# barc4/barc4dip

Measured on AMD Instinct MI355X. Metric: frames/s (2048×2048 fp32) through FFT→PSD→autocorr; % HBM roofline, higher is better.
Workload: dtype f32

## Files before the change

### barc4dip_amd/csrc/b4d_colpass.hip

```cpp
#define B4D_UNIT_TAG 1
#define B4D_UNIT_PASSES 2
#include "b4d_passes.hpp"

namespace b4d {
int col_psd_ac_pass(const b4d_plan* pl, const ColArgs& a, int batch, hipStream_t st) {
    return dispatch_col<COL_PSD_AC>(pl, a, batch, st);
}
}
```

### barc4dip_amd/csrc/b4d_common.hpp

```cpp
#pragma once
#include <hip/hip_runtime.h>

#include <atomic>
#include <mutex>
#include <string>

#include "../../include/b4d.h"

namespace b4d {

std::string& last_error();
inline int fail(int code, const std::string& msg) {
    last_error() = msg;
    return code;
}
int get_scratch(size_t bytes, void** out, hipStream_t stream);
std::recursive_mutex& scratch_mutex();
#define B4D_SCRATCH_LOCK() std::lock_guard<std::recursive_mutex> b4d_scratch_lk__(::b4d::scratch_mutex())

extern std::atomic<int> g_opt_track_predict;
extern std::atomic<int> g_opt_lanes;
extern std::atomic<int> g_opt_exp;

int ensure_dynamic_lds(const void* kernel, size_t bytes);
int lane_stream(int idx, hipStream_t* out);

#define B4D_HIP(call)                                                                      \
    do {                                                                                   \
        hipError_t e__ = (call);                                                           \
        if (e__ != hipSuccess)                                                             \
            return ::b4d::fail(B4D_EHIP, std::string(#call) + ": " + hipGetErrorString(e__)); \
    } while (0)

}
```

### barc4dip_amd/csrc/b4d_fft2d.hpp

```cpp
#pragma once
#include <hip/hip_runtime.h>

#include <algorithm>
#include <cmath>
#include <cstdint>
#include <mutex>
#include <string>
#include <vector>

#include "../../include/b4d.h"
#include "b4d_common.hpp"
#include "b4d_fft.hpp"
#include "b4d_peak.hpp"

#ifndef B4D_UNIT_TAG
#define B4D_UNIT_TAG 0
#endif
#define B4D_PASS_R2C 1
#define B4D_PASS_COL 2
#define B4D_PASS_NYQ 4
#define B4D_PASS_C2R 8
#ifndef B4D_UNIT_PASSES
#define B4D_UNIT_PASSES (B4D_PASS_R2C | B4D_PASS_COL | B4D_PASS_NYQ | B4D_PASS_C2R)
#endif
// ... 28 lines not shown
        c.x *= inv;
        c.y *= inv;
    }
    return c;
}

struct RowSrc {
    int frame, y0, y1, x0, x1;
    float mean, denom;
    int pad;
};

#ifndef B4D_K1_ITER
#define B4D_K1_ITER 1
#endif
template <int NX, int SEQ, bool SRC, int ITER = 1>
__global__ void __launch_bounds__((NX / E16) * SEQ)
k_row_r2c(const float* __restrict__ in, float2* __restrict__ spec, float* __restrict__ nyq_rows,
          const float2* __restrict__ tw, int ny, int ct_w, const RowSrc* __restrict__ srcs) {
    using G = RowGeom<NX>;
    constexpr int T = G::T, E = E16;
    constexpr bool WV = T <= 64;
    static_assert(ITER == 1 || !SRC, "ROI sources run one group per workgroup");
    __shared__ float2 lds_all[SEQ * G::LDS_ELEMS];
    const int seq = threadIdx.x / T, u = threadIdx.x % T;
    const size_t frame = blockIdx.y;
    if (SRC) {
        const int wa = 2 * blockIdx.x * SEQ, wb = wa + 2 * SEQ;
        if (wb <= srcs[frame].y0 || wa >= srcs[frame].y1) return;
    }
    float2* lds = lds_all + seq * G::LDS_ELEMS;
    float2 va[ITER][E];
#pragma unroll
    for (int it = 0; it < ITER; ++it) {
        float2(&v)[E] = va[it];
        const int pair = (blockIdx.x * ITER + it) * SEQ + seq;
        const bool live = 2 * pair < ny;
        if (!live) {
// ... 2 lines not shown
        } else if (SRC) {
            const RowSrc sd = srcs[frame];
            const int ya = 2 * pair, yb = ya + 1;
            const bool ina = ya >= sd.y0 && ya < sd.y1, inb = yb >= sd.y0 && yb < sd.y1;
            const float* r0 = in + ((size_t)sd.frame * ny + ya) * NX;
            const float* r1 = r0 + NX;
            const float inv = 1.0f / sd.denom;
#pragma unroll
            for (int j = 0; j < E; ++j) {
                const int x = u + T * j;
                const bool inx = x >= sd.x0 && x < sd.x1;
                v[j].x = (ina && inx) ? (r0[x] - sd.mean) * inv : 0.f;
                v[j].y = (inb && inx) ? (r1[x] - sd.mean) * inv : 0.f;
            }
        } else {
            const float* r0 = in + (frame * ny + 2 * (size_t)pair) * NX;
            const float* r1 = r0 + NX;
#pragma unroll
            for (int j = 0; j < E; ++j) v[j] = make_float2(r0[u + T * j], r1[u + T * j]);
        }
    }
    const int nt = (NX / 2) / ct_w;
#pragma unroll
    for (int it = 0; it < ITER; ++it) {
        float2(&v)[E] = va[it];
        const int pair = (blockIdx.x * ITER + it) * SEQ + seq;
        const bool live = 2 * pair < ny;
        if (it > 0) fft_sync<WV>();
        Fft3<G, 1, WV>::run(v, v, u, 0, lds, tw);
        fft_sync<WV>();
#pragma unroll
        for (int j = 0; j < E; ++j) lds[u + T * j] = v[j];
        fft_sync<WV>();
        if (live) {
#pragma unroll
            for (int j = 0; j < E / 2; ++j) {
                const int k = u + T * j;
                const float2 z = v[j], zr = lds[(NX - k) & (NX - 1)];
                float2 a = make_float2(0.5f * (z.x + zr.x), 0.5f * (z.y - zr.y));
                float2 b = make_float2(0.5f * (z.y + zr.y), 0.5f * (zr.x - z.x));
                if (k == 0) {
                    const float2 zn = lds[NX / 2];
                    a = make_float2(z.x, 0.f);
                    b = make_float2(z.y, 0.f);
                    nyq_rows[frame * ny + 2 * pair] = zn.x;
                    nyq_rows[frame * ny + 2 * pair + 1] = zn.y;
                }
                const size_t o = spec_index(frame, nt, ny, ct_w, 2 * pair, k);
                spec[o] = a;
                spec[o + ct_w] = b;
            }
        }
    }
}

enum ColMode { COL_PSD_AC = 0, COL_FORWARD = 2 };

struct ColArgs {
    float2* spec;
    float* psd;
    const float2* tw;
    const float2* tw_inv;
    float psd_scale;
    int nx;
    unsigned flags;
// ... 11 lines not shown
        unsigned long long t__;                                                                   \
        asm volatile("s_memtime %0\n\ts_waitcnt lgkmcnt(0)" : "=s"(t__)::"memory");              \
        __builtin_amdgcn_sched_barrier(0);                                                        \
        if (p.diag && threadIdx.x == 0) p.diag[((size_t)blockIdx.y * gridDim.x + blockIdx.x) * 8 + (i)] = t__; \
    } while (0)
#ifdef B4D_DIAG_DRAIN
#define B4D_DRAIN() asm volatile("s_waitcnt vmcnt(0)" ::: "memory")
#else
#define B4D_DRAIN() do {} while (0)
#endif
#else
#define B4D_STAMP(i) do {} while (0)
#define B4D_DRAIN() do {} while (0)
#endif

template <int NY, int SPLIT = 1>
struct ColCfg {
    static constexpr int NC = 2;
    static constexpr int CPT = (NY == 4096 ? 4 : 8) / SPLIT;
    static constexpr int CT = NC * CPT * SPLIT;
    static constexpr int THREADS = CPT * (NY / E16);
    static constexpr int WAVES_PER_EU = THREADS >= 256 ? 4 : 1;
    using G = ColGeom<NY, CPT>;
    static constexpr int SB = 1;
    static constexpr size_t LDS_BYTES = sizeof(float2) * (size_t)G::LDS_ELEMS * CPT * SB;
    static constexpr bool SERIAL = true;
};

struct __attribute__((packed, aligned(4))) float4_u {
    float x, y, z, w;
};

typedef float f32x2 __attribute__((ext_vector_type(2)));
typedef float f32x4 __attribute__((ext_vector_type(4)));
// ... 13 lines not shown
}

template <int NC>
__device__ __forceinline__ void store_cols(f32x2 B4D_GLOBAL* rowp, const float2 (&c)[NC]) {
#pragma unroll
    for (int h = 0; h < NC / 2; ++h)
        *(f32x4 B4D_GLOBAL*)(rowp + 2 * h) = f32x4{c[2 * h].x, c[2 * h].y, c[2 * h + 1].x, c[2 * h + 1].y};
}
template <int NC>
__device__ __forceinline__ void store_cols(float2* __restrict__ rowp, const float2 (&c)[NC]) {
#pragma unroll
    for (int h = 0; h < NC / 2; ++h)
        *reinterpret_cast<float4*>(rowp + 2 * h) = make_float4(c[2 * h].x, c[2 * h].y, c[2 * h + 1].x, c[2 * h + 1].y);
}

template <int NY, int MODE, int SPLIT = 1, int UNIT = 0>
__global__ void __launch_bounds__((ColCfg<NY, SPLIT>::THREADS), (ColCfg<NY, SPLIT>::WAVES_PER_EU)) k_col(ColArgs p) {
    using Cfg = ColCfg<NY, SPLIT>;
    using G = typename Cfg::G;
    constexpr int T = G::T, E = E16, NC = Cfg::NC, CPT = Cfg::CPT, CT = Cfg::CT;
    extern __shared__ __attribute__((aligned(16))) float2 lds[];
    const int cp = threadIdx.x % CPT, u = threadIdx.x / CPT;
    const int nt = gridDim.x / SPLIT;
    int slot, fr;
    if (gridDim.y % 8 == 0) {
        const unsigned lin = blockIdx.x + gridDim.x * blockIdx.y, k = lin / 8;
        fr = 8 * (k / gridDim.x) + lin % 8;
        slot = k % gridDim.x;
    } else {
        slot = (nt % 8 == 0) ? (blockIdx.x % 8) * (nt * SPLIT / 8) + blockIdx.x / 8 : blockIdx.x;
        fr = blockIdx.y;
    }
    const int ct = slot / SPLIT;
    const int cpm = cp + CPT * (slot % SPLIT);
    const size_t frame = fr;
    const int nx = p.nx;
    float2* tile = p.spec + ((frame * nt + ct) * (size_t)NY) * CT;
    const unsigned toff = (unsigned)u * CT + NC * cpm;
    float2 v[NC][E];
    B4D_STAMP(0);
    int ry0 = 0, ry1 = NY;
    if (MODE == COL_FORWARD && p.srcs) {
        ry0 = p.srcs[fr].y0;
        ry1 = p.srcs[fr].y1;
    }
#pragma unroll
    for (int h = 0; h < NC / 2; ++h) {
#pragma unroll
// ... 3 lines not shown
                float4 q = *reinterpret_cast<const float4*>(tile + (size_t)kc * CT + NC * cpm + 2 * h);
                if (ky < ry0 || ky >= ry1) q = make_float4(0.f, 0.f, 0.f, 0.f);
                v[2 * h][j] = make_float2(q.x, q.y);
                v[2 * h + 1][j] = make_float2(q.z, q.w);
            } else {
                const f32x4 q = *at_bytes<f32x4>(sgpr_base(tile + (size_t)(T * j * CT) + 2 * h), toff * 8u);
                v[2 * h][j] = make_float2(q.x, q.y);
                v[2 * h + 1][j] = make_float2(q.z, q.w);
            }
        }
    }
    B4D_DRAIN();
    B4D_STAMP(1);
    Fft3<G, 1>::template run_sets<NC, Cfg::SERIAL, MODE != COL_PSD_AC, Cfg::SB>(v, u, cp, lds, p.tw);
    B4D_STAMP(2);
    const int kx0 = ct * CT + NC * cpm;

    if (MODE == COL_FORWARD) {
        unsigned toff3 = toff;
        asm volatile("" : "+v"(toff3));
#pragma unroll
        for (int j = 0; j < E; ++j) {
            float2 c[NC];
#pragma unroll
            for (int k = 0; k < NC; ++k) c[k] = v[k][j];
            store_cols<NC>(tile + (size_t)(T * j * CT) + toff3, c);
        }
        return;
    }

    const float s = p.psd_scale;
    float* psd = p.psd ? p.psd + frame * (size_t)NY * nx : nullptr;
    int uu = u;
    asm volatile("" : "+v"(uu));
    float2 w[NC / 2][E];
    constexpr int B3 = E / G::R3;
#pragma unroll
    for (int a = 0; a < B3; ++a) {
#pragma unroll
        for (int k = 0; k < NC; ++k) Fft3<G, 1>::stage3_one(v[k], a);
#pragma unroll
        for (int q = 0; q < G::R3; ++q) {
            const int j = a + B3 * q;
            const int ky = uu + T * j;
            float pw[NC];
#pragma unroll
            for (int k = 0; k < NC; ++k) pw[k] = v[k][j].x * v[k][j].x + v[k][j].y * v[k][j].y;
#ifdef B4D_EXP_PSD_TILED
            if (psd) {
                float* pt = psd + ((size_t)ct * NY + ky) * 32 + NC * cpm;
                *reinterpret_cast<float2*>(pt) = make_float2(pw[0] * s, pw[1] * s);
                *reinterpret_cast<float2*>(pt + 16) = make_float2(pw[1] * s, pw[0] * s);
            }
            if (false) {
#else
            if (psd) {
#endif
                const unsigned rd = (unsigned)((ky + NY / 2) & (NY - 1)) * nx, rm = (unsigned)((NY / 2 - ky) & (NY - 1)) * nx;
                if (NC == 4)
                    *reinterpret_cast<float4*>(&psd[rd + nx / 2 + kx0]) =
                        make_float4(pw[0] * s, pw[1] * s, pw[2 % NC] * s, pw[3 % NC] * s);
                else
                    *at_bytes<f32x2>(psd, (rd + nx / 2 + kx0) * 4u) = f32x2{pw[0] * s, pw[1] * s};
                if (NC == 4 && kx0 >= 1) {
                    float4_u m;
                    m.x = pw[3 % NC] * s;
                    m.y = pw[2 % NC] * s;
                    m.z = pw[1] * s;
                    m.w = pw[0] * s;
                    *reinterpret_cast<float4_u*>(&psd[rm + nx / 2 - kx0 - 3]) = m;
                } else {
#if defined(B4D_EXP_NOMIRROR)
#elif defined(B4D_EXP_ALIGNED_MIRROR)
// ... 7 lines not shown
                    if (cpm == 0 && kx0 >= 1) psd[rm + nx / 2 - kx0] = pw[0] * s;
#else
                    const unsigned mo = (rm + nx / 2 - kx0 - 1) * 4u;
                    *at_bytes<float>(psd, mo) = pw[1] * s;
                    if (kx0 >= 1) *at_bytes<float>(psd, mo + 4u) = pw[0] * s;
#endif
                }
            }
#pragma unroll
            for (int h = 0; h < NC / 2; ++h) w[h][j] = make_float2(pw[2 * h + 1], pw[2 * h]);
        }
    }
    B4D_STAMP(3);
    B4D_DRAIN();
    B4D_STAMP(4);
    if (kx0 == 0 && uu == 0 && (p.flags & B4D_REMOVE_MEAN)) w[0][0].y = 0.f;
    const float2* tw2 = p.tw_inv;
    int tid2 = threadIdx.x;
    asm volatile("" : "+v"(tid2));
    const int cp2 = tid2 % CPT, u2 = tid2 / CPT;
    const unsigned toff2 = (unsigned)u2 * CT + NC * (cp2 + CPT * (slot % SPLIT));
    __syncthreads();
    Fft3<G, 1>::template run_sets<NC / 2, Cfg::SERIAL, true, Cfg::SB>(w, u2, cp2, lds, tw2);
    B4D_STAMP(5);
    float2 vr[NC / 2][E];
    constexpr int SETE = G::LDS_ELEMS * CPT;
#pragma unroll
    for (int b = 0; b < NC / 2; b += Cfg::SB) {
        __syncthreads();
#pragma unroll
        for (int h = b; h < b + Cfg::SB; ++h)
// ... 2 lines not shown
        __syncthreads();
#pragma unroll
        for (int h = b; h < b + Cfg::SB; ++h)
#pragma unroll
            for (int j = 0; j < E; ++j) vr[h][j] = lds[(h - b) * SETE + ((NY - (u2 + T * j)) & (NY - 1)) * CPT + cp2];
    }
#pragma unroll
    for (int j = 0; j < E; ++j) {
        float2 c[NC];
#pragma unroll
        for (int h = 0; h < NC / 2; ++h) {
            const float2 z = make_float2(w[h][j].y, w[h][j].x), zr = vr[h][j];
            c[2 * h] = make_float2(0.5f * (z.x + zr.x), 0.5f * (z.y - zr.y));
            c[2 * h + 1] = make_float2(0.5f * (z.y + zr.y), 0.5f * (zr.x - z.x));
        }
        if (!p.half_rows || u2 + T * j <= NY / 2 + 1) {
            static_assert(NC == 2, "one 16-byte store per row");
            __builtin_nontemporal_store(f32x4{c[0].x, c[0].y, c[1].x, c[1].y},
                                        (f32x4 B4D_GLOBAL*)at_bytes<f32x2>(sgpr_base(tile + (size_t)(T * j * CT)), toff2 * 8u));
        }
    }
    B4D_STAMP(6);
    B4D_DRAIN();
    B4D_STAMP(7);
}

enum NyqMode { NYQ_PSD_AC = 0, NYQ_FORWARD = 2, NYQ_PROD = 3, NYQ_PROD_WHITEN = 4 };

struct NyqArgs {
    const float* rows;
    float2* f_out;
// ... 76 lines not shown
    const float2* tw;
    float scale;
    int ny, ct_w;
    unsigned flags;
    float* part_val;
    int* part_idx;
    unsigned* selw;
    int sel_stride;
    unsigned pred_bin;
    float* compact;
    int half;
    int nomap;
    int nblk;
    const unsigned* gate;
    int gate_stride;
};

enum RowOutMode { C2R_OUT = 0, C2R_PEAK = 1, C2R_MAG = 2, C2R_ROWS = 3 };

template <int NX, int SEQ, int MODE, int UNIT = 0>
__global__ void __launch_bounds__((NX / E16) * SEQ) k_row_c2r(RowOutArgs p) {
    using G = RowGeom<NX>;
    constexpr int T = G::T, E = E16;
    constexpr bool WV = T <= 64;
    __shared__ float2 lds_all[SEQ * G::LDS_ELEMS];
    const int seq = threadIdx.x / T, u = threadIdx.x % T;
    const size_t frame = blockIdx.y;
    const int ny = p.ny, ct_w = p.ct_w, nt = (NX / 2) / ct_w;
    if (MODE == C2R_MAG && p.gate && p.gate[frame * p.gate_stride]) return;
    int peak_pair = 0;
    if (MODE == C2R_ROWS) {
        float bv = -1.0f;
        int bi = 0x7fffffff;
        for (int i = threadIdx.x; i < p.nblk; i += T * SEQ) argmax_merge(bv, bi, p.part_val[frame * p.nblk + i], p.part_idx[frame * p.nblk + i]);
#pragma unroll
        for (int o = 32; o > 0; o >>= 1) {
// ... 7 lines not shown
            sv[threadIdx.x >> 6] = bv;
            si[threadIdx.x >> 6] = bi;
        }
        __syncthreads();
        bv = sv[0];
        bi = si[0];
        for (int i = 1; i < (T * SEQ + 63) / 64; ++i) argmax_merge(bv, bi, sv[i], si[i]);
        __syncthreads();
        const int yr = bi == 0x7fffffff ? 0 : bi / NX;
        peak_pair = ((yr + ny / 2) & (ny - 1)) >> 1;
    }
    const int nblk = gridDim.x, bx = blockIdx.x;
    const int pair = MODE == C2R_PEAK   ? 0
                     : MODE == C2R_ROWS ? (peak_pair + ny / 2 - 1 + min(bx * SEQ + seq, 2)) % (ny / 2)
                                        : bx * SEQ + seq;
    const bool live = (MODE == C2R_OUT && p.half) ? 2 * pair <= ny / 2 : 2 * pair < ny;
    const int yl = live ? 2 * pair : 0;
    float2* lds = lds_all + seq * G::LDS_ELEMS;
    float2 v[E];
#pragma unroll
    for (int j = 0; j < E / 2; ++j) {
        const int k = u + T * j;
        const size_t o = MODE == C2R_MAG ? spec_index_pow2(frame, nt, ny, ct_w, yl, k) : spec_index(frame, nt, ny, ct_w, yl, k);
        const f32x2 a_ = __builtin_nontemporal_load(reinterpret_cast<const f32x2*>(p.g + o)),
                    b_ = __builtin_nontemporal_load(reinterpret_cast<const f32x2*>(p.g + o + ct_w));
        const float2 a = make_float2(a_.x, a_.y), b = make_float2(b_.x, b_.y);
        if (k == 0) {
            v[j] = make_float2(b.x, a.x);
            lds[NX / 2] = make_float2(p.gnyq[frame * ny + yl + 1], p.gnyq[frame * ny + yl]);
        } else {
            v[j] = make_float2(a.y + b.x, a.x - b.y);
            lds[NX - k] = make_float2(b.x - a.y, a.x + b.y);
        }
    }
    fft_sync<WV>();
#pragma unroll
    for (int j = E / 2; j < E; ++j) v[j] = lds[u + T * j];
    fft_sync<WV>();
    Fft3<G, 1, WV>::run(v, v, u, 0, lds, p.tw);
    if (MODE == C2R_PEAK) {
        if (threadIdx.x == 0) p.peak[frame] = v[0].y;
        return;
    }
    const int y0 = 2 * pair;
    const int ra = (y0 + ny / 2) & (ny - 1), rb = (y0 + 1 + ny / 2) & (ny - 1);
    float* o0 = p.out + (frame * ny + ra) * (size_t)NX;
    float* o1 = p.out + (frame * ny + rb) * (size_t)NX;
    if (MODE == C2R_OUT) {
        if (!live) return;
        const bool norm = (p.flags & B4D_NORM_PEAK) != 0;
        float s = p.scale;
        bool unit_peak = false;
        if (norm) {
            const float pk = p.peak[frame];
            unit_peak = pk > 0.f;
            s = unit_peak ? 1.0f / pk : p.scale;
        }
        const bool wr1 = !p.half || y0 + 1 <= ny / 2;
        const bool mir0 = p.half && y0 >= 1 && y0 < ny / 2, mir1 = p.half && y0 + 1 < ny / 2;
        float* q0 = p.out + (frame * ny + ((ny / 2 - y0) & (ny - 1))) * (size_t)NX;
        float* q1 = p.out + (frame * ny + ((ny / 2 - y0 - 1) & (ny - 1))) * (size_t)NX;
#pragma unroll
        for (int j = 0; j < E; ++j) {
            const int x = u + T * j, c = (x + NX / 2) & (NX - 1), cm = (NX / 2 - x) & (NX - 1);
            float r0 = v[j].y * s;
            const float r1 = v[j].x * s;
            if (unit_peak && pair == 0 && x == 0) r0 = 1.0f;
            __builtin_nontemporal_store(r0, o0 + c);
            if (wr1) __builtin_nontemporal_store(r1, o1 + c);
            if (mir0) __builtin_nontemporal_store(r0, q0 + cm);
            if (mir1) __builtin_nontemporal_store(r1, q1 + cm);
        }
        return;
    }
    if (MODE == C2R_ROWS) {
#pragma unroll
// ... 105 lines not shown
        const unsigned total = hl[2 * NW + 1];
        float* dst = p.compact + frame * (size_t)ny * NX + hl[NW];
        for (unsigned i = threadIdx.x; i < total; i += T * SEQ) dst[i] = stg[i];
    }
}

}

using namespace b4d;

struct b4d_plan {
    std::recursive_mutex mu;
    int ny, nx, chunk, ct_w;
    float2* tw_x = nullptr;
    float2* tw_y = nullptr;
    float2* spec = nullptr;
    float* nyq_rows = nullptr;
    float* gnyq = nullptr;
    float* peak = nullptr;
    size_t ws_bytes = 0;
    void* track_ws = nullptr;
    size_t track_bytes = 0;
    bool general = false;
    float2* wx = nullptr;
    float2* wy = nullptr;
    float2* gbuf1 = nullptr;
    float2* gbuf2 = nullptr;
    float2* gbuf3 = nullptr;
    bool large = false;
    bool wmr = false;
// ... 75 lines not shown
#ifndef B4D_COL_SPLIT
#define B4D_COL_SPLIT 1
#endif
template <int NY, int MODE>
static int launch_col(const ColArgs& a, int ntiles, int batch, hipStream_t st) {
    constexpr int SPLIT = (NY == 2048 && MODE == COL_PSD_AC) ? B4D_COL_SPLIT : 1;
    using Cfg = ColCfg<NY, SPLIT>;
    {
        const int rc_lds = ensure_dynamic_lds(reinterpret_cast<const void*>(&k_col<NY, MODE, SPLIT, B4D_UNIT_TAG>), Cfg::LDS_BYTES);
        if (rc_lds) return rc_lds;
    }
    hipLaunchKernelGGL((k_col<NY, MODE, SPLIT, B4D_UNIT_TAG>), dim3(ntiles * SPLIT, batch), dim3(Cfg::THREADS), Cfg::LDS_BYTES, st, a);
    B4D_HIP(hipGetLastError());
    return B4D_OK;
}
template <int MODE>
static int dispatch_col(const b4d_plan* pl, const ColArgs& a, int batch, hipStream_t st) {
    const int ntiles = (pl->nx / 2) / pl->ct_w;
#define B4D_CALL(N) launch_col<N, MODE>(a, ntiles, batch, st)
    B4D_SIZE_SWITCH(pl->ny, B4D_CALL)
#undef B4D_CALL
    return fail(B4D_ESIZE, "unsupported ny");
}
#endif

#if B4D_UNIT_PASSES & B4D_PASS_NYQ
template <int NY, int MODE>
static int launch_nyq(const NyqArgs& a, hipStream_t st) {
    constexpr int SEQ = row_seq(NY);
    hipLaunchKernelGGL((k_nyq<NY, SEQ, MODE>), dim3((a.items + SEQ - 1) / SEQ), dim3((NY / E16) * SEQ), 0, st, a);
// ... 9 lines not shown
    B4D_SIZE_SWITCH(pl->ny, B4D_CALL)
#undef B4D_CALL
    return fail(B4D_ESIZE, "unsupported ny");
}
#endif

#if B4D_UNIT_PASSES & B4D_PASS_R2C
template <int NX>
static int launch_r2c(const b4d_plan* pl, const float* in, float2* spec, float* nyq_rows, const RowSrc* srcs, int batch,
                      hipStream_t st) {
    constexpr int SEQ = row_seq(NX);
    constexpr int ITER = NX >= 1024 ? B4D_K1_ITER : 1;
    const dim3 block((NX / E16) * SEQ);
    if (srcs)
        hipLaunchKernelGGL((k_row_r2c<NX, SEQ, true>), dim3((pl->ny / 2 + SEQ - 1) / SEQ, batch), block, 0, st, in, spec, nyq_rows,
                           pl->tw_x, pl->ny, pl->ct_w, srcs);
    else
        hipLaunchKernelGGL((k_row_r2c<NX, SEQ, false, ITER>), dim3((pl->ny / 2 + SEQ * ITER - 1) / (SEQ * ITER), batch), block, 0, st,
                           in, spec, nyq_rows, pl->tw_x, pl->ny, pl->ct_w, srcs);
    B4D_HIP(hipGetLastError());
    return B4D_OK;
}
static int dispatch_r2c(const b4d_plan* pl, const float* in, int batch, hipStream_t st, float2* spec = nullptr,
                        float* nyq_rows = nullptr, const RowSrc* srcs = nullptr) {
    if (!spec) spec = pl->spec;
    if (!nyq_rows) nyq_rows = pl->nyq_rows;
#define B4D_CALL(N) launch_r2c<N>(pl, in, spec, nyq_rows, srcs, batch, st)
    B4D_SIZE_SWITCH(pl->nx, B4D_CALL)
#undef B4D_CALL
    return fail(B4D_ESIZE, "unsupported nx");
}
#endif

#if B4D_UNIT_PASSES & B4D_PASS_C2R
template <int NX>
static int launch_c2r(const b4d_plan* pl, const RowOutArgs& a, int batch, int mode, hipStream_t st,
// ... 15 lines not shown
    }
    if (a.flags & B4D_NORM_PEAK) {
        hipLaunchKernelGGL((k_row_c2r<NX, SEQ, C2R_PEAK, B4D_UNIT_TAG>), dim3(1, batch), block, 0, st, a);
        B4D_HIP(hipGetLastError());
        if (ev) {
            hipEvent_t e;
            B4D_HIP(hipEventCreate(&e));
            ev->push_back(e);
            B4D_HIP(hipEventRecord(e, st));
        }
    }
    hipLaunchKernelGGL((k_row_c2r<NX, SEQ, C2R_OUT, B4D_UNIT_TAG>), grid, block, 0, st, a);
    B4D_HIP(hipGetLastError());
    return B4D_OK;
}
static int dispatch_c2r(const b4d_plan* pl, const RowOutArgs& a, int batch, hipStream_t st, int mode = C2R_OUT,
                        std::vector<hipEvent_t>* ev = nullptr, int* nblk = nullptr) {
#define B4D_CALL(N) launch_c2r<N>(pl, a, batch, mode, st, ev, nblk)
    B4D_SIZE_SWITCH(pl->nx, B4D_CALL)
#undef B4D_CALL
    return fail(B4D_ESIZE, "unsupported nx");
}
#endif
```

### barc4dip_amd/csrc/b4d_kernels.hip

```cpp
#include "b4d_passes.hpp"
#include "b4d_wiener_mr.hpp"

#include <cstring>

namespace b4d {
std::string& last_error() {
    static thread_local std::string err;
    return err;
}
int ensure_dynamic_lds(const void* kernel, size_t bytes) {
    struct Done {
        const void* kernel;
        int dev;
        size_t bytes;
    };
    static std::mutex mu;
    static std::vector<Done> done;
    int dev = 0;
    B4D_HIP(hipGetDevice(&dev));
    std::lock_guard<std::mutex> lk(mu);
    for (Done& d : done)
        if (d.kernel == kernel && d.dev == dev) {
            if (d.bytes >= bytes) return B4D_OK;
            B4D_HIP(hipFuncSetAttribute(kernel, hipFuncAttributeMaxDynamicSharedMemorySize, (int)bytes));
// ... 17 lines not shown
    std::lock_guard<std::mutex> lk(mu);
    for (const Made& m : made)
        if (m.dev == dev && m.idx == idx) {
            *out = m.st;
            return B4D_OK;
        }
    hipStream_t st = nullptr;
    B4D_HIP(hipStreamCreateWithFlags(&st, hipStreamNonBlocking));
    made.push_back(Made{dev, idx, st});
    *out = st;
    return B4D_OK;
}
std::atomic<int> g_opt_track_predict{1};
std::atomic<int> g_opt_lanes{1};
std::atomic<int> g_opt_exp{0};
int spectrum_rows_last(const b4d_plan* pl, float2* spec, const float* frames, int batch, float2* out, hipStream_t st);
}

int Lanes::open(b4d_plan* p, hipStream_t s, int batch, size_t inter_bytes, size_t frame_bytes, bool allow_two, size_t min_group_bytes) {
    pl = p;
    st = s;
    const int want = (int)std::max<size_t>(1, ((size_t)64 << 20) / std::max<size_t>(1, inter_bytes));
    two = allow_two && b4d::g_opt_lanes.load() != 0 && batch >= 2 && p->chunk >= 2 && (size_t)batch * frame_bytes >= 2 * min_group_bytes &&
          (size_t)std::min(want, p->chunk / 2) * frame_bytes >= min_group_bytes;
    sub = two ? std::min(want, p->chunk / 2) : p->chunk;
    if (two) {
        int groups = (batch + sub - 1) / sub;
        groups += groups & 1;
        sub = (batch + groups - 1) / groups;
    }
// ... 25 lines not shown

namespace b4d {
}

extern "C" {

const char* b4d_version(void) { return "b4d 0.3.0 (gfx950)" B4D_VERSION_SUFFIX; }
const char* b4d_last_error(void) { return last_error().c_str(); }
int b4d_set_option(const char* name, int value) {
    if (!name) return fail(B4D_EINVAL, "null option name");
    struct Opt {
        const char* name;
        std::atomic<int>* v;
        int lo, hi;
    };
    const Opt opts[] = {{"track_predict_bin", &g_opt_track_predict, 0, 2}, {"lanes", &g_opt_lanes, 0, 1}, {"exp", &g_opt_exp, 0, 255}};
    for (const Opt& o : opts)
        if (!strcmp(name, o.name)) {
            if (value < o.lo || value > o.hi)
                return fail(B4D_EINVAL, std::string(name) + " takes " + std::to_string(o.lo) + " .. " + std::to_string(o.hi));
            o.v->store(value);
            return B4D_OK;
        }
    return fail(B4D_EINVAL, std::string("unknown option: ") + name);
}
static bool large_ok(int ny, int nx) {
    return ny >= 2 && nx >= 2 && ny <= 8192 && nx <= 8192 && (size_t)ny * nx <= ((size_t)1 << 26) && pm_supported(ny) && pm_supported(nx);
}
int b4d_size_supported(int ny, int nx) {
    return (pow2_ok(ny) && pow2_ok(nx)) || (general_ok(ny) && general_ok(nx)) || large_ok(ny, nx);
}
// ... 46 lines not shown
        }
        p->ws_bytes = 3 * sizeof(float2) * (size_t)chunk * ny * nx;
        hipError_t e = hipMalloc((void**)&p->gbuf1, p->ws_bytes / 3);
        if (e == hipSuccess) e = hipMalloc((void**)&p->gbuf2, p->ws_bytes / 3);
        if (e == hipSuccess) e = hipMalloc((void**)&p->gbuf3, p->ws_bytes / 3);
        if (e != hipSuccess) {
            b4d_plan_destroy(p);
            return fail(B4D_ENOMEM, std::string("workspace allocation failed: ") + hipGetErrorString(e));
        }
        *out = p;
        return B4D_OK;
    }
    p->ct_w = col_ct(ny);
    int rc = make_twiddles(nx, &p->tw_x);
    if (rc == B4D_OK) rc = make_twiddles(ny, &p->tw_y);
    if (rc != B4D_OK) {
        b4d_plan_destroy(p);
        return rc;
    }
    p->ws_bytes = sizeof(float2) * (size_t)chunk * ny * (nx / 2);
    hipError_t e = hipMalloc((void**)&p->spec, p->ws_bytes);
    if (e == hipSuccess) e = hipMalloc((void**)&p->nyq_rows, sizeof(float) * (size_t)chunk * ny);
    if (e == hipSuccess) e = hipMalloc((void**)&p->gnyq, sizeof(float) * (size_t)chunk * ny);
    if (e == hipSuccess) e = hipMalloc((void**)&p->peak, sizeof(float) * chunk);
    if (e != hipSuccess) {
        b4d_plan_destroy(p);
        return fail(B4D_ENOMEM, std::string("workspace allocation failed: ") + hipGetErrorString(e));
    }
    *out = p;
    return B4D_OK;
}

int b4d_plan_destroy(b4d_plan* p) {
    if (!p) return B4D_OK;
    if (p->tw_x) (void)hipFree(p->tw_x);
    if (p->tw_y) (void)hipFree(p->tw_y);
    if (p->spec) (void)hipFree(p->spec);
    if (p->peak) (void)hipFree(p->peak);
    if (p->nyq_rows) (void)hipFree(p->nyq_rows);
    if (p->gnyq) (void)hipFree(p->gnyq);
    if (p->track_ws) (void)hipFree(p->track_ws);
    if (p->aux) (void)hipStreamSynchronize(p->aux);
    if (p->ev_fork) (void)hipEventDestroy(p->ev_fork);
    if (p->ev_join) (void)hipEventDestroy(p->ev_join);
    for (float2* q : {p->wx, p->wy, p->gbuf1, p->gbuf2, p->gbuf3})
        if (q) (void)hipFree(q);
    delete p;
    return B4D_OK;
}

size_t b4d_plan_workspace_bytes(const b4d_plan* p) { return p ? p->ws_bytes : 0; }

#ifdef B4D_DIAG
static unsigned long long* g_diag = nullptr;
extern "C" void b4d_debug_set_diag(void* buf) { g_diag = static_cast<unsigned long long*>(buf); }
#endif

static int psd_autocorr_impl(b4d_plan* pl, const float* frames, int batch, float* psd, float psd_scale,
                             float* autocorr, unsigned flags, hipStream_t st, float* kernel_ms) {
    if (!pl) return fail(B4D_EINVAL, "plan is null");
    B4D_PLAN_LOCK(pl);
    if (!pl || !frames) return fail(B4D_EINVAL, "null plan or input");
    if (batch < 1) return fail(B4D_EINVAL, "batch must be >= 1");
    if (!psd && !autocorr) return fail(B4D_EINVAL, "both outputs are null");
    if (pl->general) return general_psd_autocorr(pl, frames, batch, psd, psd_scale, autocorr, flags, st);
    const size_t fpix = (size_t)pl->ny * pl->nx;
    std::vector<hipEvent_t> ev;
    auto mark = [&]() -> int {
        if (!kernel_ms) return B4D_OK;
        hipEvent_t e;
        B4D_HIP(hipEventCreate(&e));
        ev.push_back(e);
        B4D_HIP(hipEventRecord(e, st));
        return B4D_OK;
    };
    int rc = B4D_OK;
    Lanes ln;
    if ((rc = ln.fork(pl, st, !kernel_ms && fpix >= (size_t)4096 * 4096 && pl->chunk >= 2 && batch >= 2))) return rc;
    ln.sub = ln.two ? std::max(1, std::min(pl->chunk / 2, (batch + 1) / 2)) : pl->chunk;
    const size_t half = fpix / 2;
    int grp = 0;
    for (int b0 = 0; b0 < batch && rc == B4D_OK; b0 += ln.sub, ++grp) {
        const int nb = std::min(ln.sub, batch - b0);
        const size_t so = (size_t)ln.slot(grp) * ln.sub;
        hipStream_t ls = ln.stream(grp);
        float2* spec = pl->spec + half * so;
        float* nyq_rows = pl->nyq_rows + (size_t)pl->ny * so;
        float* gnyq = pl->gnyq + (size_t)pl->ny * so;
        if ((rc = mark())) break;
        if ((rc = dispatch_r2c(pl, frames + b0 * fpix, nb, ls, spec, nyq_rows))) break;
        if ((rc = mark())) break;
        ColArgs ca{};
        ca.spec = spec;
        ca.psd = psd ? psd + b0 * fpix : nullptr;
        ca.tw = pl->tw_y;
        ca.tw_inv = pl->tw_y;
        ca.psd_scale = psd_scale;
        ca.nx = pl->nx;
        ca.flags = flags;
        ca.half_rows = autocorr ? 1 : 0;
#ifdef B4D_DIAG
        ca.diag = g_diag;
#endif
        if ((rc = col_psd_ac_pass(pl, ca, nb, ls))) break;
        NyqArgs na{};
        na.rows = nyq_rows;
        na.g_out = gnyq;
        na.psd = ca.psd;
        na.psd_scale = psd_scale;
        if ((rc = dispatch_nyq<NYQ_PSD_AC>(pl, na, nb, ls))) break;
        if ((rc = mark())) break;
        if (autocorr) {
            RowOutArgs ra{};
            ra.g = spec;
            ra.gnyq = gnyq;
            ra.out = autocorr + b0 * fpix;
            ra.peak = pl->peak + so;
            ra.tw = pl->tw_x;
            ra.scale = 1.0f / ((float)pl->nx * (float)pl->ny);
            ra.ny = pl->ny;
            ra.ct_w = pl->ct_w;
            ra.flags = flags;
            ra.half = 1;
            if ((rc = row_out_pass(pl, ra, nb, ls, kernel_ms ? &ev : nullptr))) break;
        }
        if ((rc = mark())) break;
    }
    {
        const int rj = ln.close();
        if (rc == B4D_OK) rc = rj;
    }
    if (kernel_ms && rc == B4D_OK && !ev.empty()) {
        hipError_t e = hipEventSynchronize(ev.back());
        if (e != hipSuccess) rc = fail(B4D_EHIP, std::string("hipEventSynchronize: ") + hipGetErrorString(e));
        const bool has_peak = autocorr && (flags & B4D_NORM_PEAK);
        const size_t per = 4 + (has_peak ? 1 : 0);
        for (size_t i = 0; rc == B4D_OK && i + per <= ev.size(); i += per) {
            float ms = 0.f;
            (void)hipEventElapsedTime(&ms, ev[i], ev[i + 1]);
// ... 124 lines not shown
```

### barc4dip_amd/csrc/b4d_passes.hpp

```cpp
#pragma once
#include <vector>

#include "b4d_fft2d.hpp"

namespace b4d {
int col_psd_ac_pass(const b4d_plan* pl, const ColArgs& a, int batch, hipStream_t st);
int row_out_pass(const b4d_plan* pl, const RowOutArgs& a, int batch, hipStream_t st, std::vector<hipEvent_t>* ev);
}
```

### barc4dip_amd/csrc/b4d_rowout.hip

```cpp
#define B4D_UNIT_TAG 2
#define B4D_UNIT_PASSES 8
#include "b4d_passes.hpp"

namespace b4d {
int row_out_pass(const b4d_plan* pl, const RowOutArgs& a, int batch, hipStream_t st, std::vector<hipEvent_t>* ev) {
    return dispatch_c2r(pl, a, batch, st, C2R_OUT, ev);
}
}
```

Before: 45560.

## Split 2048-point column FFT into even/odd 1024-point halves fused into row passes

For ny=2048, the row R2C kernel pairs rows y and y+ny/2 and applies the first radix-2 decimation-in-frequency butterfly with twiddles, so the column pass only runs two independent 1024-point FFTs per column (parity tiles). The C2R row-out pass undoes the last butterfly when it loads the spectrum. The aim is to cut column-FFT LDS footprint and register pressure so the column kernel can fit more columns per workgroup. The cost is extra complex arithmetic and twiddle loads in both row kernels, plus a more complex indexing and Nyquist/mirror layout that only works for ny=2048.

```diff
diff --git a/barc4dip_amd/csrc/b4d_colpass.hip b/barc4dip_amd/csrc/b4d_colpass.hip
--- a/barc4dip_amd/csrc/b4d_colpass.hip
+++ b/barc4dip_amd/csrc/b4d_colpass.hip
@@ -3,7 +3,8 @@
 #include "b4d_passes.hpp"
 
 namespace b4d {
-int col_psd_ac_pass(const b4d_plan* pl, const ColArgs& a, int batch, hipStream_t st) {
+int col_psd_ac_pass(const b4d_plan* pl, const ColArgs& a, int batch, hipStream_t st, int ysplit) {
+    if (ysplit) return launch_col_ys(pl, a, batch, st);
     return dispatch_col<COL_PSD_AC>(pl, a, batch, st);
 }
 }
diff --git a/barc4dip_amd/csrc/b4d_common.hpp b/barc4dip_amd/csrc/b4d_common.hpp
--- a/barc4dip_amd/csrc/b4d_common.hpp
+++ b/barc4dip_amd/csrc/b4d_common.hpp
@@ -20,6 +20,7 @@
 
 extern std::atomic<int> g_opt_track_predict;
 extern std::atomic<int> g_opt_lanes;
+extern std::atomic<int> g_opt_ysplit;
 extern std::atomic<int> g_opt_exp;
 
 int ensure_dynamic_lds(const void* kernel, size_t bytes);
diff --git a/barc4dip_amd/csrc/b4d_fft2d.hpp b/barc4dip_amd/csrc/b4d_fft2d.hpp
--- a/barc4dip_amd/csrc/b4d_fft2d.hpp
+++ b/barc4dip_amd/csrc/b4d_fft2d.hpp
@@ -66,14 +66,15 @@
 #ifndef B4D_K1_ITER
 #define B4D_K1_ITER 1
 #endif
-template <int NX, int SEQ, bool SRC, int ITER = 1>
+template <int NX, int SEQ, bool SRC, int ITER = 1, bool YS = false>
 __global__ void __launch_bounds__((NX / E16) * SEQ)
 k_row_r2c(const float* __restrict__ in, float2* __restrict__ spec, float* __restrict__ nyq_rows,
-          const float2* __restrict__ tw, int ny, int ct_w, const RowSrc* __restrict__ srcs) {
+          const float2* __restrict__ tw, int ny, int ct_w, const RowSrc* __restrict__ srcs, const float2* __restrict__ tw_y) {
     using G = RowGeom<NX>;
     constexpr int T = G::T, E = E16;
     constexpr bool WV = T <= 64;
     static_assert(ITER == 1 || !SRC, "ROI sources run one group per workgroup");
+    static_assert(!YS || !SRC, "the ysplit pairing takes full frames");
     __shared__ float2 lds_all[SEQ * G::LDS_ELEMS];
     const int seq = threadIdx.x / T, u = threadIdx.x % T;
     const size_t frame = blockIdx.y;
@@ -106,8 +107,8 @@
                 v[j].y = (inb && inx) ? (r1[x] - sd.mean) * inv : 0.f;
             }
         } else {
-            const float* r0 = in + (frame * ny + 2 * (size_t)pair) * NX;
-            const float* r1 = r0 + NX;
+            const float* r0 = in + (frame * ny + (YS ? 1 : 2) * (size_t)pair) * NX;
+            const float* r1 = r0 + (YS ? (size_t)(ny / 2) * NX : (size_t)NX);
 #pragma unroll
             for (int j = 0; j < E; ++j) v[j] = make_float2(r0[u + T * j], r1[u + T * j]);
         }
@@ -125,6 +126,8 @@
         for (int j = 0; j < E; ++j) lds[u + T * j] = v[j];
         fft_sync<WV>();
         if (live) {
+            float2 wp = make_float2(1.f, 0.f);
+            if (YS) wp = tw_y[pair];
 #pragma unroll
             for (int j = 0; j < E / 2; ++j) {
                 const int k = u + T * j;
@@ -135,12 +138,18 @@
                     const float2 zn = lds[NX / 2];
                     a = make_float2(z.x, 0.f);
                     b = make_float2(z.y, 0.f);
-                    nyq_rows[frame * ny + 2 * pair] = zn.x;
-                    nyq_rows[frame * ny + 2 * pair + 1] = zn.y;
+                    nyq_rows[frame * ny + (YS ? pair : 2 * pair)] = zn.x;
+                    nyq_rows[frame * ny + (YS ? pair + ny / 2 : 2 * pair + 1)] = zn.y;
                 }
-                const size_t o = spec_index(frame, nt, ny, ct_w, 2 * pair, k);
-                spec[o] = a;
-                spec[o + ct_w] = b;
+                if (YS) {
+                    const size_t o = spec_index(2 * frame, nt, ny / 2, ct_w, pair, k);
+                    spec[o] = cadd(a, b);
+                    spec[o + (size_t)(ny / 2) * (NX / 2)] = cmul(csub(a, b), wp);
+                } else {
+                    const size_t o = spec_index(frame, nt, ny, ct_w, 2 * pair, k);
+                    spec[o] = a;
+                    spec[o + ct_w] = b;
+                }
             }
         }
     }
@@ -182,10 +191,10 @@
 #define B4D_DRAIN() do {} while (0)
 #endif
 
-template <int NY, int SPLIT = 1>
+template <int NY, int SPLIT = 1, int YS = 0>
 struct ColCfg {
     static constexpr int NC = 2;
-    static constexpr int CPT = (NY == 4096 ? 4 : 8) / SPLIT;
+    static constexpr int CPT = (NY == 4096 ? 4 : 8) / SPLIT * (YS ? 2 : 1);
     static constexpr int CT = NC * CPT * SPLIT;
     static constexpr int THREADS = CPT * (NY / E16);
     static constexpr int WAVES_PER_EU = THREADS >= 256 ? 4 : 1;
@@ -229,9 +238,11 @@
         *reinterpret_cast<float4*>(rowp + 2 * h) = make_float4(c[2 * h].x, c[2 * h].y, c[2 * h + 1].x, c[2 * h + 1].y);
 }
 
-template <int NY, int MODE, int SPLIT = 1, int UNIT = 0>
-__global__ void __launch_bounds__((ColCfg<NY, SPLIT>::THREADS), (ColCfg<NY, SPLIT>::WAVES_PER_EU)) k_col(ColArgs p) {
-    using Cfg = ColCfg<NY, SPLIT>;
+template <int NY, int MODE, int SPLIT = 1, int UNIT = 0, int YS = 0>
+__global__ void __launch_bounds__((ColCfg<NY, SPLIT, YS>::THREADS), (ColCfg<NY, SPLIT, YS>::WAVES_PER_EU)) k_col(ColArgs p) {
+    using Cfg = ColCfg<NY, SPLIT, YS>;
+    static_assert(YS == 0 || (MODE == COL_PSD_AC && SPLIT == 1), "parity tiles: fused PSD + autocorrelation pass only");
+    constexpr int NYF = YS ? 2 * NY : NY;
     using G = typename Cfg::G;
     constexpr int T = G::T, E = E16, NC = Cfg::NC, CPT = Cfg::CPT, CT = Cfg::CT;
     extern __shared__ __attribute__((aligned(16))) float2 lds[];
@@ -247,6 +258,8 @@
         fr = blockIdx.y;
     }
     const int ct = slot / SPLIT;
+    const int par = (YS && ct >= nt / 2) ? 1 : 0;
+    const int ctx = YS ? ct - par * (nt / 2) : ct;
     const int cpm = cp + CPT * (slot % SPLIT);
     const size_t frame = fr;
     const int nx = p.nx;
@@ -280,7 +293,7 @@
     B4D_STAMP(1);
     Fft3<G, 1>::template run_sets<NC, Cfg::SERIAL, MODE != COL_PSD_AC, Cfg::SB>(v, u, cp, lds, p.tw);
     B4D_STAMP(2);
-    const int kx0 = ct * CT + NC * cpm;
+    const int kx0 = ctx * CT + NC * cpm;
 
     if (MODE == COL_FORWARD) {
         unsigned toff3 = toff;
@@ -296,7 +309,7 @@
     }
 
     const float s = p.psd_scale;
-    float* psd = p.psd ? p.psd + frame * (size_t)NY * nx : nullptr;
+    float* psd = p.psd ? p.psd + frame * (size_t)NYF * nx : nullptr;
     int uu = u;
     asm volatile("" : "+v"(uu));
     float2 w[NC / 2][E];
@@ -308,13 +321,13 @@
 #pragma unroll
         for (int q = 0; q < G::R3; ++q) {
             const int j = a + B3 * q;
-            const int ky = uu + T * j;
+            const int ky = YS ? 2 * (uu + T * j) + par : uu + T * j;
             float pw[NC];
 #pragma unroll
             for (int k = 0; k < NC; ++k) pw[k] = v[k][j].x * v[k][j].x + v[k][j].y * v[k][j].y;
 #ifdef B4D_EXP_PSD_TILED
             if (psd) {
-                float* pt = psd + ((size_t)ct * NY + ky) * 32 + NC * cpm;
+                float* pt = psd + ((size_t)ctx * NYF + ky) * 32 + NC * cpm;
                 *reinterpret_cast<float2*>(pt) = make_float2(pw[0] * s, pw[1] * s);
                 *reinterpret_cast<float2*>(pt + 16) = make_float2(pw[1] * s, pw[0] * s);
             }
@@ -322,7 +335,7 @@
 #else
             if (psd) {
 #endif
-                const unsigned rd = (unsigned)((ky + NY / 2) & (NY - 1)) * nx, rm = (unsigned)((NY / 2 - ky) & (NY - 1)) * nx;
+                const unsigned rd = (unsigned)((ky + NYF / 2) & (NYF - 1)) * nx, rm = (unsigned)((NYF / 2 - ky) & (NYF - 1)) * nx;
                 if (NC == 4)
                     *reinterpret_cast<float4*>(&psd[rd + nx / 2 + kx0]) =
                         make_float4(pw[0] * s, pw[1] * s, pw[2 % NC] * s, pw[3 % NC] * s);
@@ -360,7 +373,7 @@
     B4D_STAMP(3);
     B4D_DRAIN();
     B4D_STAMP(4);
-    if (kx0 == 0 && uu == 0 && (p.flags & B4D_REMOVE_MEAN)) w[0][0].y = 0.f;
+    if (kx0 == 0 && uu == 0 && par == 0 && (p.flags & B4D_REMOVE_MEAN)) w[0][0].y = 0.f;
     const float2* tw2 = p.tw_inv;
     int tid2 = threadIdx.x;
     asm volatile("" : "+v"(tid2));
@@ -393,7 +406,7 @@
             c[2 * h] = make_float2(0.5f * (z.x + zr.x), 0.5f * (z.y - zr.y));
             c[2 * h + 1] = make_float2(0.5f * (z.y + zr.y), 0.5f * (zr.x - z.x));
         }
-        if (!p.half_rows || u2 + T * j <= NY / 2 + 1) {
+        if (!p.half_rows || u2 + T * j <= (YS ? NY / 2 : NY / 2 + 1)) {
             static_assert(NC == 2, "one 16-byte store per row");
             __builtin_nontemporal_store(f32x4{c[0].x, c[0].y, c[1].x, c[1].y},
                                         (f32x4 B4D_GLOBAL*)at_bytes<f32x2>(sgpr_base(tile + (size_t)(T * j * CT)), toff2 * 8u));
@@ -500,12 +513,14 @@
     int nblk;
     const unsigned* gate;
     int gate_stride;
+    const float2* tw_y;
 };
 
 enum RowOutMode { C2R_OUT = 0, C2R_PEAK = 1, C2R_MAG = 2, C2R_ROWS = 3 };
 
-template <int NX, int SEQ, int MODE, int UNIT = 0>
+template <int NX, int SEQ, int MODE, int UNIT = 0, bool YS = false>
 __global__ void __launch_bounds__((NX / E16) * SEQ) k_row_c2r(RowOutArgs p) {
+    static_assert(!YS || MODE == C2R_OUT || MODE == C2R_PEAK, "ysplit: autocorrelation output only");
     using G = RowGeom<NX>;
     constexpr int T = G::T, E = E16;
     constexpr bool WV = T <= 64;
@@ -543,13 +558,33 @@
     const int pair = MODE == C2R_PEAK   ? 0
                      : MODE == C2R_ROWS ? (peak_pair + ny / 2 - 1 + min(bx * SEQ + seq, 2)) % (ny / 2)
                                         : bx * SEQ + seq;
-    const bool live = (MODE == C2R_OUT && p.half) ? 2 * pair <= ny / 2 : 2 * pair < ny;
-    const int yl = live ? 2 * pair : 0;
+    const bool live = YS ? 4 * pair <= ny : (MODE == C2R_OUT && p.half) ? 2 * pair <= ny / 2 : 2 * pair < ny;
+    const int yl = live ? (YS ? pair : 2 * pair) : 0;
     float2* lds = lds_all + seq * G::LDS_ELEMS;
     float2 v[E];
+    float2 wc = make_float2(1.f, 0.f);
+    if (YS) {
+        wc = p.tw_y[yl];
+        wc.y = -wc.y;
+    }
 #pragma unroll
     for (int j = 0; j < E / 2; ++j) {
         const int k = u + T * j;
+        if (YS) {
+            const size_t o = spec_index(2 * frame, nt, ny / 2, ct_w, yl, k);
+            const f32x2 e_ = __builtin_nontemporal_load(reinterpret_cast<const f32x2*>(p.g + o)),
+                        o_ = __builtin_nontemporal_load(reinterpret_cast<const f32x2*>(p.g + o + (size_t)(ny / 2) * (NX / 2)));
+            const float2 ev = make_float2(e_.x, e_.y), t = cmul(make_float2(o_.x, o_.y), wc);
+            const float2 a = cadd(ev, t), d = csub(ev, t), b = make_float2(d.x, -d.y);
+            if (k == 0) {
+                v[j] = make_float2(b.x, a.x);
+                lds[NX / 2] = make_float2(p.gnyq[frame * ny + ny / 2 - yl], p.gnyq[frame * ny + yl]);
+            } else {
+                v[j] = make_float2(a.y + b.x, a.x - b.y);
+                lds[NX - k] = make_float2(b.x - a.y, a.x + b.y);
+            }
+            continue;
+        }
         const size_t o = MODE == C2R_MAG ? spec_index_pow2(frame, nt, ny, ct_w, yl, k) : spec_index(frame, nt, ny, ct_w, yl, k);
         const f32x2 a_ = __builtin_nontemporal_load(reinterpret_cast<const f32x2*>(p.g + o)),
                     b_ = __builtin_nontemporal_load(reinterpret_cast<const f32x2*>(p.g + o + ct_w));
@@ -571,8 +606,9 @@
         if (threadIdx.x == 0) p.peak[frame] = v[0].y;
         return;
     }
-    const int y0 = 2 * pair;
-    const int ra = (y0 + ny / 2) & (ny - 1), rb = (y0 + 1 + ny / 2) & (ny - 1);
+    const int y0 = YS ? pair : 2 * pair;
+    const int y1 = YS ? ny / 2 - pair : y0 + 1;
+    const int ra = (y0 + ny / 2) & (ny - 1), rb = (y1 + ny / 2) & (ny - 1);
     float* o0 = p.out + (frame * ny + ra) * (size_t)NX;
     float* o1 = p.out + (frame * ny + rb) * (size_t)NX;
     if (MODE == C2R_OUT) {
@@ -585,10 +621,10 @@
             unit_peak = pk > 0.f;
             s = unit_peak ? 1.0f / pk : p.scale;
         }
-        const bool wr1 = !p.half || y0 + 1 <= ny / 2;
-        const bool mir0 = p.half && y0 >= 1 && y0 < ny / 2, mir1 = p.half && y0 + 1 < ny / 2;
+        const bool wr1 = YS ? 4 * y0 < ny : !p.half || y0 + 1 <= ny / 2;
+        const bool mir0 = YS ? y0 >= 1 : p.half && y0 >= 1 && y0 < ny / 2, mir1 = YS ? y0 >= 1 && 4 * y0 < ny : p.half && y0 + 1 < ny / 2;
         float* q0 = p.out + (frame * ny + ((ny / 2 - y0) & (ny - 1))) * (size_t)NX;
-        float* q1 = p.out + (frame * ny + ((ny / 2 - y0 - 1) & (ny - 1))) * (size_t)NX;
+        float* q1 = p.out + (frame * ny + ((ny / 2 - y1) & (ny - 1))) * (size_t)NX;
 #pragma unroll
         for (int j = 0; j < E; ++j) {
             const int x = u + T * j, c = (x + NX / 2) & (NX - 1), cm = (NX / 2 - x) & (NX - 1);
@@ -724,6 +760,7 @@
     int ny, nx, chunk, ct_w;
     float2* tw_x = nullptr;
     float2* tw_y = nullptr;
+    float2* tw_yh = nullptr;
     float2* spec = nullptr;
     float* nyq_rows = nullptr;
     float* gnyq = nullptr;
@@ -829,6 +866,19 @@
     B4D_HIP(hipGetLastError());
     return B4D_OK;
 }
+template <int YS = 1>
+static int launch_col_ys(const b4d_plan* pl, const ColArgs& a, int batch, hipStream_t st) {
+    using Cfg = ColCfg<1024, 1, YS>;
+    if (pl->ny != 2048 || (pl->nx / 2) % Cfg::CT) return fail(B4D_ESIZE, "ysplit column pass: unsupported size");
+    {
+        const int rc_lds = ensure_dynamic_lds(reinterpret_cast<const void*>(&k_col<1024, COL_PSD_AC, 1, B4D_UNIT_TAG, YS>), Cfg::LDS_BYTES);
+        if (rc_lds) return rc_lds;
+    }
+    hipLaunchKernelGGL((k_col<1024, COL_PSD_AC, 1, B4D_UNIT_TAG, YS>), dim3(2 * ((pl->nx / 2) / Cfg::CT), batch), dim3(Cfg::THREADS),
+                       Cfg::LDS_BYTES, st, a);
+    B4D_HIP(hipGetLastError());
+    return B4D_OK;
+}
 template <int MODE>
 static int dispatch_col(const b4d_plan* pl, const ColArgs& a, int batch, hipStream_t st) {
     const int ntiles = (pl->nx / 2) / pl->ct_w;
@@ -868,12 +918,28 @@
     const dim3 block((NX / E16) * SEQ);
     if (srcs)
         hipLaunchKernelGGL((k_row_r2c<NX, SEQ, true>), dim3((pl->ny / 2 + SEQ - 1) / SEQ, batch), block, 0, st, in, spec, nyq_rows,
-                           pl->tw_x, pl->ny, pl->ct_w, srcs);
+                           pl->tw_x, pl->ny, pl->ct_w, srcs, (const float2*)nullptr);
     else
         hipLaunchKernelGGL((k_row_r2c<NX, SEQ, false, ITER>), dim3((pl->ny / 2 + SEQ * ITER - 1) / (SEQ * ITER), batch), block, 0, st,
-                           in, spec, nyq_rows, pl->tw_x, pl->ny, pl->ct_w, srcs);
+                           in, spec, nyq_rows, pl->tw_x, pl->ny, pl->ct_w, srcs, (const float2*)nullptr);
     B4D_HIP(hipGetLastError());
     return B4D_OK;
+}
+template <int NX>
+static int launch_r2c_ys(const b4d_plan* pl, const float* in, float2* spec, float* nyq_rows, int ct_w, int batch, hipStream_t st) {
+    constexpr int SEQ = row_seq(NX);
+    constexpr int ITER = NX >= 1024 ? B4D_K1_ITER : 1;
+    hipLaunchKernelGGL((k_row_r2c<NX, SEQ, false, ITER, true>), dim3((pl->ny / 2 + SEQ * ITER - 1) / (SEQ * ITER), batch),
+                       dim3((NX / E16) * SEQ), 0, st, in, spec, nyq_rows, pl->tw_x, pl->ny, ct_w, (const RowSrc*)nullptr, pl->tw_y);
+    B4D_HIP(hipGetLastError());
+    return B4D_OK;
+}
+template <int DUMMY = 0>
+static int dispatch_r2c_ys(const b4d_plan* pl, const float* in, int batch, hipStream_t st, float2* spec, float* nyq_rows, int ct_w) {
+#define B4D_CALL(N) launch_r2c_ys<N>(pl, in, spec, nyq_rows, ct_w, batch, st)
+    B4D_SIZE_SWITCH(pl->nx, B4D_CALL)
+#undef B4D_CALL
+    return fail(B4D_ESIZE, "unsupported nx");
 }
 static int dispatch_r2c(const b4d_plan* pl, const float* in, int batch, hipStream_t st, float2* spec = nullptr,
                         float* nyq_rows = nullptr, const RowSrc* srcs = nullptr) {
@@ -919,6 +985,32 @@
     B4D_HIP(hipGetLastError());
     return B4D_OK;
 }
+template <int NX>
+static int launch_c2r_ys(const b4d_plan* pl, const RowOutArgs& a, int batch, hipStream_t st, std::vector<hipEvent_t>* ev) {
+    constexpr int SEQ = row_seq(NX);
+    const dim3 grid((pl->ny / 4 + 1 + SEQ - 1) / SEQ, batch), block((NX / E16) * SEQ);
+    if (batch < 1) return B4D_OK;
+    if (a.flags & B4D_NORM_PEAK) {
+        hipLaunchKernelGGL((k_row_c2r<NX, SEQ, C2R_PEAK, B4D_UNIT_TAG, true>), dim3(1, batch), block, 0, st, a);
+        B4D_HIP(hipGetLastError());
+        if (ev) {
+            hipEvent_t e;
+            B4D_HIP(hipEventCreate(&e));
+            ev->push_back(e);
+            B4D_HIP(hipEventRecord(e, st));
+        }
+    }
+    hipLaunchKernelGGL((k_row_c2r<NX, SEQ, C2R_OUT, B4D_UNIT_TAG, true>), grid, block, 0, st, a);
+    B4D_HIP(hipGetLastError());
+    return B4D_OK;
+}
+template <int DUMMY = 0>
+static int dispatch_c2r_ys(const b4d_plan* pl, const RowOutArgs& a, int batch, hipStream_t st, std::vector<hipEvent_t>* ev) {
+#define B4D_CALL(N) launch_c2r_ys<N>(pl, a, batch, st, ev)
+    B4D_SIZE_SWITCH(pl->nx, B4D_CALL)
+#undef B4D_CALL
+    return fail(B4D_ESIZE, "unsupported nx");
+}
 static int dispatch_c2r(const b4d_plan* pl, const RowOutArgs& a, int batch, hipStream_t st, int mode = C2R_OUT,
                         std::vector<hipEvent_t>* ev = nullptr, int* nblk = nullptr) {
 #define B4D_CALL(N) launch_c2r<N>(pl, a, batch, mode, st, ev, nblk)
diff --git a/barc4dip_amd/csrc/b4d_kernels.hip b/barc4dip_amd/csrc/b4d_kernels.hip
--- a/barc4dip_amd/csrc/b4d_kernels.hip
+++ b/barc4dip_amd/csrc/b4d_kernels.hip
@@ -55,6 +55,7 @@
 std::atomic<int> g_opt_track_predict{1};
 std::atomic<int> g_opt_lanes{1};
 std::atomic<int> g_opt_exp{0};
+std::atomic<int> g_opt_ysplit{1};
 int spectrum_rows_last(const b4d_plan* pl, float2* spec, const float* frames, int batch, float2* out, hipStream_t st);
 }
 
@@ -110,7 +111,8 @@
         std::atomic<int>* v;
         int lo, hi;
     };
-    const Opt opts[] = {{"track_predict_bin", &g_opt_track_predict, 0, 2}, {"lanes", &g_opt_lanes, 0, 1}, {"exp", &g_opt_exp, 0, 255}};
+    const Opt opts[] = {{"track_predict_bin", &g_opt_track_predict, 0, 2}, {"lanes", &g_opt_lanes, 0, 1}, {"exp", &g_opt_exp, 0, 255},
+                        {"ysplit", &g_opt_ysplit, 0, 1}};
     for (const Opt& o : opts)
         if (!strcmp(name, o.name)) {
             if (value < o.lo || value > o.hi)
@@ -187,6 +189,7 @@
     p->ct_w = col_ct(ny);
     int rc = make_twiddles(nx, &p->tw_x);
     if (rc == B4D_OK) rc = make_twiddles(ny, &p->tw_y);
+    if (rc == B4D_OK && ny == 2048) rc = make_twiddles(ny / 2, &p->tw_yh);
     if (rc != B4D_OK) {
         b4d_plan_destroy(p);
         return rc;
@@ -208,6 +211,7 @@
     if (!p) return B4D_OK;
     if (p->tw_x) (void)hipFree(p->tw_x);
     if (p->tw_y) (void)hipFree(p->tw_y);
+    if (p->tw_yh) (void)hipFree(p->tw_yh);
     if (p->spec) (void)hipFree(p->spec);
     if (p->peak) (void)hipFree(p->peak);
     if (p->nyq_rows) (void)hipFree(p->nyq_rows);
@@ -238,6 +242,8 @@
     if (!psd && !autocorr) return fail(B4D_EINVAL, "both outputs are null");
     if (pl->general) return general_psd_autocorr(pl, frames, batch, psd, psd_scale, autocorr, flags, st);
     const size_t fpix = (size_t)pl->ny * pl->nx;
+    const int ysplit = (pl->ny == 2048 && pl->tw_yh) ? g_opt_ysplit.load() : 0;
+    constexpr int ys_ct = ColCfg<1024, 1, 1>::CT;
     std::vector<hipEvent_t> ev;
     auto mark = [&]() -> int {
         if (!kernel_ms) return B4D_OK;
@@ -261,13 +267,15 @@
         float* nyq_rows = pl->nyq_rows + (size_t)pl->ny * so;
         float* gnyq = pl->gnyq + (size_t)pl->ny * so;
         if ((rc = mark())) break;
-        if ((rc = dispatch_r2c(pl, frames + b0 * fpix, nb, ls, spec, nyq_rows))) break;
+        if ((rc = ysplit ? dispatch_r2c_ys(pl, frames + b0 * fpix, nb, ls, spec, nyq_rows, ys_ct)
+                         : dispatch_r2c(pl, frames + b0 * fpix, nb, ls, spec, nyq_rows)))
+            break;
         if ((rc = mark())) break;
         ColArgs ca{};
         ca.spec = spec;
         ca.psd = psd ? psd + b0 * fpix : nullptr;
-        ca.tw = pl->tw_y;
-        ca.tw_inv = pl->tw_y;
+        ca.tw = ysplit ? pl->tw_yh : pl->tw_y;
+        ca.tw_inv = ca.tw;
         ca.psd_scale = psd_scale;
         ca.nx = pl->nx;
         ca.flags = flags;
@@ -275,7 +283,7 @@
 #ifdef B4D_DIAG
         ca.diag = g_diag;
 #endif
-        if ((rc = col_psd_ac_pass(pl, ca, nb, ls))) break;
+        if ((rc = col_psd_ac_pass(pl, ca, nb, ls, ysplit))) break;
         NyqArgs na{};
         na.rows = nyq_rows;
         na.g_out = gnyq;
@@ -292,10 +300,11 @@
             ra.tw = pl->tw_x;
             ra.scale = 1.0f / ((float)pl->nx * (float)pl->ny);
             ra.ny = pl->ny;
-            ra.ct_w = pl->ct_w;
+            ra.ct_w = ysplit ? ys_ct : pl->ct_w;
+            ra.tw_y = pl->tw_y;
             ra.flags = flags;
             ra.half = 1;
-            if ((rc = row_out_pass(pl, ra, nb, ls, kernel_ms ? &ev : nullptr))) break;
+            if ((rc = row_out_pass(pl, ra, nb, ls, kernel_ms ? &ev : nullptr, ysplit))) break;
         }
         if ((rc = mark())) break;
     }
diff --git a/barc4dip_amd/csrc/b4d_passes.hpp b/barc4dip_amd/csrc/b4d_passes.hpp
--- a/barc4dip_amd/csrc/b4d_passes.hpp
+++ b/barc4dip_amd/csrc/b4d_passes.hpp
@@ -4,6 +4,6 @@
 #include "b4d_fft2d.hpp"
 
 namespace b4d {
-int col_psd_ac_pass(const b4d_plan* pl, const ColArgs& a, int batch, hipStream_t st);
-int row_out_pass(const b4d_plan* pl, const RowOutArgs& a, int batch, hipStream_t st, std::vector<hipEvent_t>* ev);
+int col_psd_ac_pass(const b4d_plan* pl, const ColArgs& a, int batch, hipStream_t st, int ysplit);
+int row_out_pass(const b4d_plan* pl, const RowOutArgs& a, int batch, hipStream_t st, std::vector<hipEvent_t>* ev, int ysplit);
 }
diff --git a/barc4dip_amd/csrc/b4d_rowout.hip b/barc4dip_amd/csrc/b4d_rowout.hip
--- a/barc4dip_amd/csrc/b4d_rowout.hip
+++ b/barc4dip_amd/csrc/b4d_rowout.hip
@@ -3,7 +3,8 @@
 #include "b4d_passes.hpp"
 
 namespace b4d {
-int row_out_pass(const b4d_plan* pl, const RowOutArgs& a, int batch, hipStream_t st, std::vector<hipEvent_t>* ev) {
+int row_out_pass(const b4d_plan* pl, const RowOutArgs& a, int batch, hipStream_t st, std::vector<hipEvent_t>* ev, int ysplit) {
+    if (ysplit) return dispatch_c2r_ys(pl, a, batch, st, ev);
     return dispatch_c2r(pl, a, batch, st, C2R_OUT, ev);
 }
 }
```

After: 47280, median of 6. 3.8% higher.
